# suilin0432/SoS-WSOD

Measured on AMD Instinct MI355X. Metric: images/s (1/2/4/8 MI355X) VGG16+OICR 2000-prop; conv5_3 MFMA-util %, higher is better.
Workload: dtype bf16; 1 GPU; OICR+ training iteration: 4 views/step/GPU (1 image(s) x 2 scales x h-flip, every view 512x512), R=2000 proposals/view, K=20, VGG16 dilated-C5 + ROIPool 7x7 + fc6/fc7 4096 + WSDDN + 4 OICR heads, fwd+bwd+SGD(momentum, wd); image=one view, parallelism=dp1

## Files before the change

### include/soswsod_hip.h

```cpp
#ifndef SOSWSOD_HIP_H
#define SOSWSOD_HIP_H

#include <stdint.h>

#ifdef __cplusplus
extern "C" {
#endif

#ifndef SW_F32
#define SW_F32 0
#define SW_BF16 1
#endif

typedef struct ihipStream_t* sw_stream_t;

typedef struct sw_epilogue {
  const float* bias;
  int relu;
  const uint8_t* drop_mask;
  long ld_drop;
  float drop_scale;
  const void* relu_ref;
  long ld_ref;
  float ref_scale;
// ... 161 lines not shown
typedef struct sw_sgd_tensor_s {
  float* param;
  const float* grad;
  float* momentum_buf;
  long n;
  float lr, weight_decay;
  int first_step;
  int stage_kind, stage_dtype;
  void* stage0;
  void* stage1;
  int d0, d1, d2;
  long ld0, ld1;
  const float* hyper_dev;
} sw_sgd_tensor;
int sw_sgd_multi(int n_tensors, const sw_sgd_tensor* tensors, float momentum, float grad_scale, sw_stream_t stream);
int sw_gemm_sgd_fused_supported(int dtype, int a_kstrided, int b_kstrided, int M, int N, int K);
int sw_loss_finalize(int n_losses, int V, int n_images, const float* loss_view, float* out, float* total,
                     sw_stream_t stream);
int sw_scale_cols_loss(int dtype, int M, int N, int n_valid, const float* in, long ld_in, const float* g_losses,
                       const float* g_total, const int32_t* col_to_loss, float mul, void* out, long ld_out,
                       sw_stream_t stream);
int sw_resize_pass_u8(int C, int H, int W, long in_ld, long in_plane, int out_size, int horizontal, const uint8_t* in,
                      const int32_t* bounds, const int32_t* kk, int ksize, uint8_t* out, uint8_t* out_flip, sw_stream_t stream);
int sw_color_jitter_u8(int H, int W, int mode, const uint8_t* in, float w_bright, double src_w_sat, float w_sat, uint8_t* out,
                       uint8_t* out_flip, sw_stream_t stream);
int sw_pack_views(int R, const float* const* box_ptrs4, const float* const* obj_ptrs4, float* boxes, float* obj,
                  float* rois, sw_stream_t stream);

int sw_preprocess_pad(int dtype, int h, int w, int H, int W, const uint8_t* img_chw, const float* mean3, const float* std3,
                      void* out_nhwc4, sw_stream_t stream);
// ... 157 lines not shown
```

### sos-wsod_amd/_lib.py

```python
import ctypes
import os

import torch

_HERE = os.path.dirname(os.path.abspath(__file__))
LIB_PATH = os.environ.get("SW_LIB_PATH") or os.path.join(_HERE, "libsoswsod_hip.so")

SW_F32, SW_BF16 = 0, 1

c_int, c_long, c_float, c_void_p, c_u64 = ctypes.c_int, ctypes.c_long, ctypes.c_float, ctypes.c_void_p, ctypes.c_uint64
c_int32, c_uint32, c_double, c_longlong = ctypes.c_int32, ctypes.c_uint32, ctypes.c_double, ctypes.c_longlong


class Epilogue(ctypes.Structure):
    _fields_ = [
        ("bias", c_void_p), ("relu", c_int), ("drop_mask", c_void_p), ("ld_drop", c_long), ("drop_scale", c_float),
        ("relu_ref", c_void_p), ("ld_ref", c_long), ("ref_scale", c_float), ("ref_dtype", c_int),
        ("out_dtype", c_int), ("accumulate_atomic", c_int), ("absmax_out", c_void_p),
        ("drop_seed", c_u64), ("drop_offset", c_u64), ("drop_hash_p", c_float), ("drop_offset_dev", c_void_p),
        ("splitk_workspace", c_void_p),
        ("residual", c_void_p), ("ld_res", c_long), ("res_dtype", c_int),
        ("fold_row_scale", c_void_p),
        ("sgd_fused", c_void_p), ("sgd_momentum", c_float), ("sgd_grad_scale", c_float),
    ]
# ... 50 lines not shown
                ("scale", c_void_p), ("shift", c_void_p), ("dst", c_void_p),
                ("kind", c_int32), ("rows", c_int32), ("cols", c_int32), ("block_start", c_int32)]


class ColsumFold(ctypes.Structure):
    _fields_ = [("N", c_int), ("n_partial_rows", c_int), ("workspace", c_void_p), ("out", c_void_p)]


class SgdTensor(ctypes.Structure):
    _fields_ = [
        ("param", c_void_p), ("grad", c_void_p), ("momentum_buf", c_void_p), ("n", c_long), ("lr", c_float),
        ("weight_decay", c_float), ("first_step", c_int), ("stage_kind", c_int), ("stage_dtype", c_int),
        ("stage0", c_void_p), ("stage1", c_void_p), ("d0", c_int), ("d1", c_int), ("d2", c_int), ("ld0", c_long), ("ld1", c_long),
        ("hyper_dev", c_void_p),
    ]


class JpegInfo(ctypes.Structure):
    _fields_ = [("width", c_int32), ("height", c_int32), ("ncomp", c_int32), ("restart_interval", c_int32),
                ("orientation", c_int32), ("mcus_x", c_int32), ("mcus_y", c_int32),
                ("hsamp", c_int32 * 3), ("vsamp", c_int32 * 3), ("qtable", c_int32 * 3),
                ("blocks_w", c_int32 * 3), ("blocks_h", c_int32 * 3), ("coef_bytes", ctypes.c_int64)]


class JpegDesc(ctypes.Structure):
    _fields_ = [("out", c_void_p), ("coef_off", ctypes.c_int64), ("qtab_off", ctypes.c_int64), ("plane_off", ctypes.c_int64),
                ("block_start", c_int32), ("quad_start", c_int32),
                ("width", c_int32), ("height", c_int32), ("ncomp", c_int32), ("hsamp", c_int32), ("vsamp", c_int32),
                ("bgr", c_int32), ("blocks_w", c_int32 * 3), ("blocks_h", c_int32 * 3), ("qtable", c_int32 * 3),
                ("pad_", c_int32)]
# ... 55 lines not shown
    "sw_splitk_fold_multi": (c_int, [c_int, ctypes.POINTER(SplitkFold), c_void_p]),
    "sw_colsum_fold_multi": (c_int, [c_int, ctypes.POINTER(ColsumFold), c_void_p]),
    "sw_colsum_partial_multi": (c_int, [c_int, c_int, ctypes.POINTER(ColsumPart), c_void_p]),
    "sw_conv3x3_wgrad_grouped": (c_int, [c_int, c_int, ctypes.POINTER(WgradProblem), c_void_p]),
    "sw_convert_2d": (c_int, [c_int, c_int, c_int, c_void_p, c_long, c_void_p, c_long, c_void_p]),
    "sw_split_bf16x3": (c_int, [c_int, c_int, c_void_p, c_long, c_void_p, c_long, c_int, c_int, c_void_p]),
    "sw_nchw_to_nhwc": (c_int, [c_int, c_int, c_int, c_int, c_int, c_int, c_void_p, c_void_p, c_void_p]),
    "sw_relu_bwd": (c_int, [c_int, c_long, c_void_p, c_void_p, c_void_p, c_void_p]),
    "sw_scale_cols": (c_int, [c_int, c_int, c_int, c_void_p, c_long, c_void_p, c_void_p, c_long, c_void_p]),
    "sw_fill_zero": (c_int, [c_void_p, c_long, c_void_p]),
    "sw_dropout_mask": (c_int, [c_void_p, c_long, c_u64, c_u64, c_float, c_void_p]),
    "sw_sgd_momentum_step": (c_int, [c_void_p, c_void_p, c_void_p, c_long, c_float, c_float, c_float, c_int, c_float,
                                     c_void_p]),
    "sw_convert_2d_t": (c_int, [c_int, c_int, c_int, c_void_p, c_long, c_void_p, c_long, c_void_p]),
    "sw_sgd_multi": (c_int, [c_int, ctypes.POINTER(SgdTensor), c_float, c_float, c_void_p]),
    "sw_loss_finalize": (c_int, [c_int, c_int, c_int, c_void_p, c_void_p, c_void_p, c_void_p]),
    "sw_scale_cols_loss": (c_int, [c_int, c_int, c_int, c_int, c_void_p, c_long, c_void_p, c_void_p, c_void_p, c_float,
                                   c_void_p, c_long, c_void_p]),
    "sw_resize_pass_u8": (c_int, [c_int, c_int, c_int, c_long, c_long, c_int, c_int, c_void_p, c_void_p, c_void_p, c_int, c_void_p,
                                  c_void_p, c_void_p]),
    "sw_color_jitter_u8": (c_int, [c_int, c_int, c_int, c_void_p, c_float, c_double, c_float, c_void_p, c_void_p, c_void_p]),
    "sw_transpose_2d": (c_int, [c_int, c_int, c_int, c_void_p, c_long, c_void_p, c_long, c_void_p]),
    "sw_stage_blocks": (c_int, [c_int, c_int, c_int]),
    "sw_stage_weights_multi": (c_int, [c_int, c_int, c_void_p, c_int, c_float, c_void_p]),
    "sw_ema_multi": (c_int, [c_int, ctypes.POINTER(c_void_p), ctypes.POINTER(c_void_p), ctypes.POINTER(c_long), c_double, c_void_p]),
    "sw_threshold_select": (c_int, [c_int, c_void_p, c_void_p, c_void_p, c_float, c_void_p, c_int, c_void_p, c_void_p, c_void_p,
                                    c_void_p, c_void_p, c_void_p]),
    "sw_conv3x3_relu_pool2": (c_int, [c_int, c_int, c_int, c_int, c_int, c_int, c_void_p, c_void_p, c_void_p, c_void_p, c_void_p]),
    "sw_weighted_sum": (c_int, [c_int, c_void_p, c_void_p, c_void_p, c_void_p]),
    "sw_scale_scalars": (c_int, [c_int, c_void_p, c_void_p, c_void_p, c_void_p]),
# ... 97 lines not shown
```

### sos-wsod_amd/backbone_vgg.py

```python
import os

import torch
import torch.nn as nn

from . import ops, staging, wgrad
from .registry import BACKBONE_REGISTRY
from .structures import ShapeSpec

_STAGES = [("plain1", 3, 64, 2), ("plain2", 64, 128, 2), ("plain3", 128, 256, 3), ("plain4", 256, 512, 3),
           ("plain5", 512, 512, 3)]


def _epc(dtype):
    return 8 if dtype == torch.bfloat16 else 4


class _Conv(nn.Module):

    def __init__(self, cin, cout):
        super().__init__()
        self.weight = nn.Parameter(torch.empty(cout, cin, 3, 3))
        self.bias = nn.Parameter(torch.zeros(cout))
        nn.init.kaiming_normal_(self.weight, mode="fan_out", nonlinearity="relu")

# ... 134 lines not shown
                w = params[pidx]
                if w.requires_grad:
                    cout = blk.out_channels
                    slab_off, row_off, nslab, nrow, splits = {}, {}, 0, 0, {}
                    for i in live:
                        x_in = infos[i][si][0][ci][0]
                        n, H, W, cin = x_in.shape
                        splits[i] = (direct_ns[(pidx, i)] if direct_ns is not None
                                     else wgrad.wgrad_grouped_splits(nmul * n * H * W, bk, target))
                        slab_off[i], row_off[i] = nslab, nrow
                        nslab += ops.conv3x3_wgrad_nslab_shape(wdt, nmul * n, H, W, cin, cout, splits[i])
                        nrow += ops.colsum_nrows(dtype, n * H * W, cout)
                    cin = infos[live[0]][si][0][ci][0].shape[3]
                    plan[pidx] = dict(ws=torch.empty(nslab, cout * 9 * cin, device=dev, dtype=torch.float32),
                                      rows=torch.empty(nrow, cout, device=dev, dtype=torch.float32), slab_off=slab_off,
                                      row_off=row_off, nslab=nslab, nrow=nrow, splits=splits, cin=cin,
                                      dw=ops.grad_target(w, (cout, cin, 3, 3), dev),
                                      db=ops.grad_target(params[pidx + 1], (cout,), dev))
                if (si, ci) == first_trainable:
                    break
            if si == first_trainable[0]:
                break
        if side is not None:
            side.wait_stream(main)
        for k, i in enumerate(live):
            st = side if (side is not None and k % 2 == 1) else main
            with torch.cuda.stream(st):
                g = gs[i]
                if st is not main:
                    g.record_stream(st)
                _VGGFunction._backward_one(module, infos[i], params, g, dtype, plan, i, first_trainable,
                                           deferred, None if st is main else main, x3w)
            infos[i] = None
        if side is not None:
            main.wait_stream(side)
        if deferred:
            ops.conv3x3_wgrad_grouped(deferred, tag="wgrad_grouped")
            ops.colsum_partial_multi(module._colsum_deferred)
            deferred.clear()
        module._colsum_deferred = []
        ops.conv3x3_wgrad_fold_multi([(pl["ws"], pl["nslab"], pl["dw"]) for pl in plan.values()])
        ops.colsum_fold_multi([(pl["rows"], pl["nrow"], pl["db"]) for pl in plan.values()])
        for pidx, pl in plan.items():
            w = params[pidx]
            grads[pidx] = pl["dw"][:, : w.shape[1]].contiguous() if pl["cin"] != w.shape[1] else pl["dw"]
            grads[pidx + 1] = pl["db"]
        return (None, None) + (None,) * n_in + tuple(grads)

    @staticmethod
    def _backward_one(module, stage_info, params, g, dtype, plan, i, first_trainable, deferred, consumer_stream, x3w=False):
        g = g.contiguous()
        if g.dtype != dtype:
            g = g.to(dtype)
        last_out = stage_info[-1][0][-1][1]
        assert stage_info[-1][1] is None, "backward expects the last stage to have no pool (vgg.py:197)"
        dz = ops.relu_bwd(last_out, g, out=torch.empty_like(g))
        pidx = len(params)
        for si in range(len(stage_info) - 1, -1, -1):
# ... 108 lines not shown
        dtype = self.compute_dtype
        epc = _epc(dtype)
        ft = self.first_trainable_conv()
        for si, blk in enumerate(self.blocks):
            for ci, c in enumerate(blk.convs()):
                cout, cin = c.weight.shape[:2]
                cin_pad = (cin + epc - 1) // epc * epc
                self.staged_weight(c.weight, 0, cin_pad, dtype)
                if self.x3_layer(dtype, cin_pad, cout):
                    self.staged_weight_x3(c.weight, 0, cin_pad)
                if with_dgrad and ft is not None and (si, ci) > ft:
                    self.staged_weight(c.weight, 1, cin, dtype)
                    if self.x3_layer(dtype, cout, cin):
                        self.staged_weight_x3(c.weight, 1, cin)

    def first_trainable_conv(self):
        for si, blk in enumerate(self.blocks):
            for ci, c in enumerate(blk.convs()):
                if c.weight.requires_grad:
                    return (si, ci)
        return None

    def _flat_params(self):
        out = []
        for blk in self.blocks:
            for c in blk.convs():
                out += [c.weight, c.bias]
        return out

    def side_stream(self):
# ... 39 lines not shown
```

### sos-wsod_amd/csrc/common.h

```cpp
#pragma once
#include <hip/hip_runtime.h>
#include <stdint.h>
#include <atomic>

#define SW_F32 0
#define SW_BF16 1

typedef __attribute__((ext_vector_type(4))) float f32x4;
typedef __attribute__((ext_vector_type(16))) float f32x16;
typedef __attribute__((ext_vector_type(8))) __bf16 bf16x8;
typedef __attribute__((ext_vector_type(4))) short s16x4;
typedef __attribute__((ext_vector_type(8))) short s16x8;
typedef __attribute__((ext_vector_type(4))) unsigned int u32x4;
typedef __attribute__((ext_vector_type(2))) unsigned int u32x2;

__device__ __forceinline__ float bf16_bits_to_f32(unsigned short b) {
  return __uint_as_float(((unsigned int)b) << 16);
}
__device__ __forceinline__ unsigned short f32_to_bf16_bits(float f) {
  __bf16 h = (__bf16)f;
  return __builtin_bit_cast(unsigned short, h);
}

template <typename T> struct Elem;
// ... 40 lines not shown
  float r = (lane < nw) ? red[lane] : 0.f;
  r = wave_reduce_sum(r);
  return r;
}
__device__ __forceinline__ float block_reduce_max(float v, float* red) {
  v = wave_reduce_max(v);
  const int lane = threadIdx.x & 63, w = threadIdx.x >> 6, nw = blockDim.x >> 6;
  __syncthreads();
  if (lane == 0) red[w] = v;
  __syncthreads();
  float r = (lane < nw) ? red[lane] : -3.402823466e38f;
  r = wave_reduce_max(r);
  return r;
}

typedef __attribute__((ext_vector_type(4))) int sw_i32x4;
__device__ __forceinline__ sw_i32x4 sw_make_rsrc(const void* base, unsigned bytes) {
  const unsigned long long b = (unsigned long long)base;
  return sw_i32x4{(int)(unsigned)b, (int)(unsigned)((b >> 32) & 0xFFFFu), (int)bytes, 0x00020000};
}
__device__ __forceinline__ void sw_dma16(const sw_i32x4 rsrc, const char* lds_dst, unsigned voff, unsigned soff) {
  const unsigned m = (unsigned)(size_t)(__attribute__((address_space(3))) const char*)lds_dst;
  asm volatile("s_mov_b32 m0, %0\n\ts_nop 0\n\tbuffer_load_dwordx4 %1, %2, %3 offen lds" ::"s"(m), "v"(voff), "s"(rsrc), "s"(soff) : "memory");
}

inline int sw_cu_count() {
  static std::atomic<int> cus[64];
  int dev = 0;
  if (hipGetDevice(&dev) != hipSuccess || dev < 0 || dev >= 64) return 256;
  int n = cus[dev].load(std::memory_order_relaxed);
// ... 14 lines not shown
```

### sos-wsod_amd/csrc/elementwise.hip

```cpp
#include "common.h"
#include "soswsod_hip.h"

namespace {

inline int grid_for(long n, int block = 256) {
  long g = (n + block - 1) / block;
  return (int)(g < 1 ? 1 : (g > 2048 ? 2048 : g));
}

template <typename T>
__global__ void preprocess_kernel(int H, int W, int cpad, const uint8_t* __restrict__ img, float m0, float m1, float m2,
                                  float s0, float s1, float s2, T* __restrict__ out) {
  const long npix = (long)H * W;
  for (long p = blockIdx.x * (long)blockDim.x + threadIdx.x; p < npix; p += (long)gridDim.x * blockDim.x) {
    const float v0 = __fdiv_rn((float)img[p] - m0, s0);
    const float v1 = __fdiv_rn((float)img[npix + p] - m1, s1);
    const float v2 = __fdiv_rn((float)img[2 * npix + p] - m2, s2);
    T* o = out + p * cpad;
    Elem<T>::store(o + 0, v0); Elem<T>::store(o + 1, v1); Elem<T>::store(o + 2, v2);
    for (int c = 3; c < cpad; ++c) Elem<T>::store(o + c, 0.f);
  }
}

constexpr int PRE_MAX = 16;
// ... 321 lines not shown
struct ColsumPartMulti {
  int n;
  int M[CPART_MAX], N[CPART_MAX], rpc[CPART_MAX], slabs[CPART_MAX], first_wg[CPART_MAX + 1];
  long ld[CPART_MAX];
  const void* X[CPART_MAX];
  float* ws[CPART_MAX];
};
template <typename T>
__global__ __launch_bounds__(256) void colsum_ws_multi_kernel(ColsumPartMulti f) {
  int i = 0;
  while (i + 1 < f.n && (int)blockIdx.x >= f.first_wg[i + 1]) ++i;
  const int w = (int)blockIdx.x - f.first_wg[i];
  colsum_ws_body<T>(f.M[i], f.N[i], f.rpc[i], (const T*)f.X[i], f.ld[i], f.ws[i], w % f.slabs[i], w / f.slabs[i]);
}

__device__ __forceinline__ void colsum_fold_body(int N, int nchunk, const float* __restrict__ ws, float* __restrict__ out, int wg,
                                                 const int accumulate = 0) {
  __shared__ float fold[16][17];
  const int tid = threadIdx.x, cl = tid >> 4, c16 = tid & 15, col = wg * 16 + c16;
  float f = 0.f;
  if (col < N)
    for (int c = cl; c < nchunk; c += 16) f += ws[(long)c * N + col];
  fold[cl][c16] = f;
  __syncthreads();
  if (cl == 0 && col < N) {
    float s = 0.f;
#pragma unroll
    for (int r = 0; r < 16; ++r) s += fold[r][c16];
    out[col] = accumulate ? out[col] + s : s;
  }
}

__global__ __launch_bounds__(256) void colsum_fold_kernel(int N, int nchunk, const float* __restrict__ ws, float* __restrict__ out, int accumulate) {
  colsum_fold_body(N, nchunk, ws, out, blockIdx.x, accumulate);
}

constexpr int CFOLD_MAX = 32;
struct ColsumFoldMulti {
  int n;
  int first_wg[CFOLD_MAX + 1];
  int N[CFOLD_MAX], rows[CFOLD_MAX];
  const float* ws[CFOLD_MAX];
  float* out[CFOLD_MAX];
};
__global__ __launch_bounds__(256) void colsum_fold_multi_kernel(ColsumFoldMulti f) {
// ... 39 lines not shown
  if (d.stage_kind == 1) {
    const long r = i / d.d0; const int c = (int)(i - r * d.d0);
    Elem<T>::store((T*)d.stage0 + r * d.ld0 + c, w);
  } else {
    const int tap = (int)(i % 9); const long t = i / 9;
    const int ci = (int)(t % d.d1); const int co = (int)(t / d.d1);
    if (d.stage0) Elem<T>::store((T*)d.stage0 + ((long)co * 9 + tap) * d.d2 + ci, w);
    if (d.stage1) Elem<T>::store((T*)d.stage1 + ((long)ci * 9 + (8 - tap)) * d.d0 + co, w);
  }
}

__device__ __forceinline__ bool sgd_conv_tileable(const sw_sgd_tensor& d) {
  return d.stage_kind == 2 && (d.d0 % 32) == 0 && (d.d1 % 32) == 0;
}

template <typename T>
__device__ __forceinline__ void sgd_conv_tile(const sw_sgd_tensor& d, int blk, float mom, float gscale, float (*tile)[289]) {
  const int cib = d.d1 / 32;
  const int co0 = (blk / cib) * 32, ci0 = (blk % cib) * 32;
  const int Cin = d.d1, Cout = d.d0;
  const float lr = d.hyper_dev ? d.hyper_dev[0] : d.lr, wd = d.hyper_dev ? d.hyper_dev[1] : d.weight_decay;
  for (int idx = threadIdx.x; idx < 32 * 288; idx += 256) {
    const int co_l = idx / 288, rem = idx - co_l * 288;
    const long o = ((long)(co0 + co_l) * Cin + ci0) * 9 + rem;
    const float w0 = d.param[o];
    const float dd = d.grad[o] * gscale + wd * w0;
    const float m = d.first_step ? dd : mom * d.momentum_buf[o] + dd;
    const float w1 = w0 - lr * m;
    d.momentum_buf[o] = m; d.param[o] = w1;
    tile[co_l][rem] = w1;
  }
  __syncthreads();
  if (d.stage0) {
// ... 731 lines not shown
      const long nb = conv_tiles ? (long)(d.d0 / 32) * (d.d1 / 32) : (d.n + SGD_CHUNK - 1) / SGD_CHUNK;
      if (nb > (1L << 30)) return -6;
      b.t[b.n] = d;
      b.block_start[b.n] = blocks;
      blocks += (int)nb;
      ++b.n;
    }
    b.block_start[b.n] = blocks;
    if (b.n == 0) continue;
    hipLaunchKernelGGL(sgd_multi_kernel, dim3(blocks), dim3(256), 0, stream, b, momentum, grad_scale);
    SW_CHECK_LAUNCH();
  }
  return 0;
}

extern "C" int sw_mean_views(int V, long n, const float* in, float* out, hipStream_t stream) {
  SW_ENTER();
  if (n <= 0) return 0;
  hipLaunchKernelGGL(mean_views_kernel, dim3(grid_for(n)), dim3(256), 0, stream, V, n, in, out);
  SW_CHECK_LAUNCH();
  return 0;
}

extern "C" int sw_loss_finalize(int n_losses, int V, int n_images, const float* loss_view, float* out, float* total,
                                hipStream_t stream) {
  SW_ENTER();
  if (n_losses > 64 || n_losses < 1 || V < 1 || n_images < 1) return -6;
  hipLaunchKernelGGL(loss_finalize_kernel, dim3(1), dim3(64), 0, stream, n_losses, V, n_images, loss_view, out, total);
  SW_CHECK_LAUNCH();
  return 0;
// ... 279 lines not shown
```

### sos-wsod_amd/csrc/gemm.hip

```cpp
#include "common.h"
#include "soswsod_hip.h"

namespace {

enum { OP_KCONTIG = 0, OP_KSTRIDED = 1, OP_CONV_A = 2, OP_CONV_B = 3, OP_CONV_A_GEN = 4 };

struct GemmArgs {
  const void* A; const void* B; void* C;
  int M, N, K;
  long lda, ldb, ldc;
  int tiles_m, tiles_n, patches_m, k_per_split;
  int patch_m_log2;
  int cH, cW, cC, cDil;
  const float* bias;
  const uint8_t* drop; long ldd; float drop_scale;
  unsigned long long drop_seed_mixed, drop_offset; float drop_p;
  const unsigned long long* drop_offset_dev;
  const void* ref; long ldr; float ref_scale; int ref_bf16;
  const void* res; long ldres; int res_bf16;
  int relu, out_bf16, atomic, oihw_cin, staged_out;
  unsigned a_bytes, b_bytes;
  long slab_stride;
  int vgrid;
  int krot;
// ... 1125 lines not shown
  return dtype == SW_BF16 ? dispatch_modes<unsigned short>(g, amode, OP_KCONTIG, 1, stream)
                          : dispatch_modes<float>(g, amode, OP_KCONTIG, 1, stream);
}

namespace {
__device__ __forceinline__ void wgrad_reduce_body(int Cout, int Cin, int nslab, const float* __restrict__ slabs,
                                                  float* __restrict__ out, int co, int parts, int part, float* s_t,
                                                  const float* __restrict__ cout_scale = nullptr, const int accumulate = 0) {
  const int CI = Cin / parts, ci0 = part * CI;
  const int cv = CI >> 2, nv = 9 * cv;
  const long slab_f = (long)Cout * 9 * Cin;
  const float* src = slabs + (long)co * 9 * Cin + ci0;
  for (int q = threadIdx.x; q < nv; q += 256) {
    const int tap = q / cv, c4 = q - tap * cv;
    const float* p = src + (long)tap * Cin + c4 * 4;
    f32x4 a0 = {0.f, 0.f, 0.f, 0.f}, a1 = a0, a2 = a0, a3 = a0;
    int z = 0;
    for (; z + 8 <= nslab; z += 8) {
      f32x4 v[8];
#pragma unroll
      for (int u = 0; u < 8; ++u) v[u] = *(const f32x4*)(p + (long)(z + u) * slab_f);
      a0 += v[0]; a1 += v[1]; a2 += v[2]; a3 += v[3];
      a0 += v[4]; a1 += v[5]; a2 += v[6]; a3 += v[7];
    }
    for (; z < nslab; ++z) a0 += *(const f32x4*)(p + (long)z * slab_f);
    f32x4 r = (a0 + a1) + (a2 + a3);
    if (cout_scale) { const float sc = cout_scale[co]; r[0] = __fmul_rn(r[0], sc); r[1] = __fmul_rn(r[1], sc); r[2] = __fmul_rn(r[2], sc); r[3] = __fmul_rn(r[3], sc); }
    *(f32x4*)(s_t + tap * CI + c4 * 4) = r;
  }
  __syncthreads();
  f32x4* dst = (f32x4*)(out + ((long)co * Cin + ci0) * 9);
  for (int q = threadIdx.x; q < nv; q += 256) {
    f32x4 o;
#pragma unroll
    for (int j = 0; j < 4; ++j) {
      const int e = 4 * q + j, ci = e / 9, tap = e - 9 * ci;
      o[j] = s_t[tap * CI + ci];
    }
    if (accumulate) o += dst[q];
    dst[q] = o;
  }
// ... 291 lines not shown
```

### sos-wsod_amd/ops.py

```python
import ctypes

import torch

from ._lib import SW_BF16, SW_F32, Epilogue, check, lib


def _p(t):
    return None if t is None else ctypes.c_void_p(t.data_ptr())


def _floats(vals, n):
    return (ctypes.c_float * n)(*[float(v) for v in vals])


def _workspace256(nbytes, device):
    ws = torch.empty(nbytes + 256, device=device, dtype=torch.uint8)
    return ws, ctypes.c_void_p((ws.data_ptr() + 255) // 256 * 256)


_raw_stream = getattr(torch._C, "_cuda_getCurrentRawStream", None)


def _stream():
    if _raw_stream is not None:
# ... 446 lines not shown
def _fill_sgd_tensor(d, e):
    p = e["param"]
    g = e.get("grad")
    d.param, d.grad, d.momentum_buf, d.n = p.data_ptr(), (None if g is None else g.data_ptr()), e["buf"].data_ptr(), p.numel()
    d.lr, d.weight_decay, d.first_step = float(e["lr"]), float(e["weight_decay"]), int(e["first"])
    hy = e.get("hyper")
    d.hyper_dev = None if hy is None else hy.data_ptr()
    st = e.get("staging")
    if st is None:
        d.stage_kind = 0
    else:
        d.stage_kind, d.stage_dtype = st["kind"], dt(st["dtype"])
        d.stage0 = None if st["stage0"] is None else st["stage0"].data_ptr()
        d.stage1 = None if st["stage1"] is None else st["stage1"].data_ptr()
        d.d0, d.d1, d.d2, d.ld0, d.ld1 = st["d0"], st["d1"], st["d2"], st["ld0"], st.get("ld1", 0)


def gemm_sgd_fused_supported(dtype, M, N, K, a_kstrided=False, b_kstrided=False):
    return bool(lib.sw_gemm_sgd_fused_supported(dt(dtype), int(a_kstrided), int(b_kstrided), int(M), int(N), int(K)))


def attach_sgd_fused(ep, entry, momentum, grad_scale=1.0):
    from ._lib import SgdTensor
    d = SgdTensor()
    _fill_sgd_tensor(d, entry)
    ep.sgd_fused = ctypes.addressof(d)
    ep.sgd_momentum, ep.sgd_grad_scale = float(momentum), float(grad_scale)
    ep._keepalive = ep._keepalive + (d, entry["param"], entry["buf"], entry.get("hyper"))
    return ep

# ... 865 lines not shown
```

### sos-wsod_amd/solver.py

```python
from bisect import bisect_right
from typing import List

import torch

from . import ops, staging


class HipSGD(torch.optim.Optimizer):

    def __init__(self, params, lr, momentum=0.0, weight_decay=0.0, device_hyper=False):
        super().__init__(params, dict(lr=lr, momentum=momentum, weight_decay=weight_decay))
        self.device_hyper = bool(device_hyper)
        self._hyper_dev = None
        self._hyper_host = None
        self._done = set()
        self._group_of = None

    def sync_hyper(self):
        if not self.device_hyper:
            return
        vals = [(float(g["lr"]), float(g["weight_decay"])) for g in self.param_groups]
        if self._hyper_dev is None:
            dev = next(p.device for g in self.param_groups for p in g["params"])
            self._hyper_dev = torch.zeros(len(vals), 2, dtype=torch.float32, device=dev)
# ... 19 lines not shown
        for i, p in enumerate(params):
            g = p.grad if grads is None else grads[i]
            ent = self._group_of.get(id(p))
            if ent is None or g is None or id(p) in self._done:
                continue
            items.append((ent[0], ent[1], p, g.view_as(p)))
            self._done.add(id(p))
        self._update(items, grad_scale)

    @torch.no_grad()
    def fused_update_entry(self, p):
        if self._group_of is None:
            self._group_of = {id(q): (group, gi) for gi, group in enumerate(self.param_groups) for q in group["params"]}
        ent = self._group_of.get(id(p))
        staged = staging.entry_of(p)
        if (ent is None or staged is None or staged["kind"] != 3 or p.dtype != torch.float32 or not p.is_contiguous()):
            return None
        group, gi = ent
        if self.device_hyper and (self._hyper_dev is None or not torch.cuda.is_current_stream_capturing()):
            self.sync_hyper()
        st = self.state[p]
        first = "momentum_buffer" not in st
        if first:
            st["momentum_buffer"] = torch.zeros_like(p, memory_format=torch.contiguous_format)
        entry = dict(param=p, buf=st["momentum_buffer"], lr=group["lr"], weight_decay=group["weight_decay"], first=first,
                     staging=staged, hyper=self._hyper_dev[gi] if self.device_hyper else None)
        return entry, float(group["momentum"]), lambda: staging.updated(p)

    def _update(self, items, grad_scale):
        if not items:
            return
# ... 67 lines not shown
```

### sos-wsod_amd/trainer.py

```python
import os
from collections import OrderedDict

import torch
import torch.distributed as dist

from .events import EventStorage


def init_distributed(backend=None):
    world = int(os.environ.get("WORLD_SIZE", "1"))
    rank = int(os.environ.get("RANK", "0"))
    local_rank = int(os.environ.get("LOCAL_RANK", "0"))
    if world > 1 and not dist.is_initialized():
        if backend is None:
            backend = "nccl" if torch.cuda.is_available() else "gloo"
        if backend == "nccl" and "SW_BENCH_DEVICE" not in os.environ:
            torch.cuda.set_device(local_rank)
        dist.init_process_group(backend=backend, rank=rank, world_size=world)
    return rank, local_rank, world


def auto_scale_workers(cfg, num_workers: int):
    import math
    old = cfg.SOLVER.REFERENCE_WORLD_SIZE
    if old == 0 or old == num_workers or old < num_workers:
        return cfg
    cfg = cfg.clone()
    scale = num_workers / old
    cfg.SOLVER.BASE_LR = cfg.SOLVER.BASE_LR / scale
    cfg.WSL.ITER_SIZE = math.ceil(cfg.WSL.ITER_SIZE / scale)
    return cfg


class Trainer:

    def __init__(self, model, optimizer, data_iter=None, iter_size=1, scheduler=None, ddp=None, find_unused=False,
                 check_finite_every=20, grad_compress=None, metrics_period=20, bucket_cap_mb=128, start_iter=0,
                 use_graph=None, overlap_update=None):
        self.raw_model = model
        self.optimizer, self.scheduler = optimizer, scheduler
        self.iter_size = max(int(iter_size), 1)
        self.data_iter = data_iter
        self.iter = self.start_iter = int(start_iter)
        self.check_finite_every = check_finite_every
        self.metrics_period = metrics_period
        self.storage = EventStorage(self.iter)
        self._finite_flag = None
        self._grad_seed = None
        if use_graph is None:
            use_graph = os.environ.get("SW_STEP_GRAPH", "0") == "1"
        self._graphs = None
        self._want_graph = bool(use_graph)
        self.world = dist.get_world_size() if (dist.is_available() and dist.is_initialized()) else 1
# ... 45 lines not shown
                    def update(fut):
                        v = fut.value()
                        opt.step_params(bucket.parameters(), bucket.gradients())
                        return v[0] if isinstance(v, (list, tuple)) else v
                    return reduce_hook(state, bucket).then(update)
                self.model.register_comm_hook(None, hook)
            else:
                self.model.register_comm_hook(None, reduce_hook)
        else:
            self.model = model
        heads = getattr(model, "roi_heads", None)
        if heads is not None and hasattr(heads, "_fused_fc1_plan"):
            fuse = (not use_ddp and self.iter_size == 1 and hasattr(optimizer, "fused_update_entry")
                    and os.environ.get("SW_FUSE_FC1_UPDATE", "1") == "1")
            heads.__dict__["_fused_opt"] = optimizer if fuse else None
        if self._want_graph and not use_ddp and self.iter_size == 1 and hasattr(model, "roi_heads") and \
                next(model.parameters()).is_cuda:
            self._graphs = _StepGraphs(self)

    def _seed_grad(self, total):
        if self._grad_seed is None or self._grad_seed.device != total.device or self._grad_seed.dtype != total.dtype:
            self._grad_seed = torch.full_like(total, getattr(self, "_seed_scale", 1.0) / self.iter_size)
        return self._grad_seed

    def _raise_if_nonfinite(self):
        if self._finite_flag is not None:
            it, flag = self._finite_flag
            self._finite_flag = None
            if not bool(flag.item()):
                raise FloatingPointError("Loss became infinite or NaN at iteration={}!".format(it))
# ... 465 lines not shown
```

Measured before the change: 499.4 images/s.

## Fuse conv weight-gradient slab fold with SGD update and bf16 weight staging

Adds a grouped kernel that reduces the split-K wgrad slabs and bias partial rows, applies momentum SGD, and writes the staged bf16 (and flipped) weight copies in one pass per 32x32 tile. This replaces the separate fold kernels, gradient materialization and later optimizer/staging passes for backbone convs when running single-GPU with iter_size 1. It also adds a wide vectorized path to the existing conv SGD tile kernel. The fused path drops the separate dw/db tensors, so parameters with existing .grad or unaligned shapes fall back to the old path.

```diff
diff --git a/include/soswsod_hip.h b/include/soswsod_hip.h
--- a/include/soswsod_hip.h
+++ b/include/soswsod_hip.h
@@ -199,6 +199,9 @@
   const float* hyper_dev;
 } sw_sgd_tensor;
 int sw_sgd_multi(int n_tensors, const sw_sgd_tensor* tensors, float momentum, float grad_scale, sw_stream_t stream);
+#define SW_CONV_FOLD_SGD_MAX_ITEMS 24
+typedef struct sw_conv_fold_sgd_item { const float* workspace; int nfold, ws_cin, kind; sw_sgd_tensor t; } sw_conv_fold_sgd_item;
+int sw_conv_fold_sgd_multi(int n, const sw_conv_fold_sgd_item* items, float momentum, float grad_scale, sw_stream_t stream);
 int sw_gemm_sgd_fused_supported(int dtype, int a_kstrided, int b_kstrided, int M, int N, int K);
 int sw_loss_finalize(int n_losses, int V, int n_images, const float* loss_view, float* out, float* total,
                      sw_stream_t stream);
diff --git a/sos-wsod_amd/_lib.py b/sos-wsod_amd/_lib.py
--- a/sos-wsod_amd/_lib.py
+++ b/sos-wsod_amd/_lib.py
@@ -88,6 +88,10 @@
         ("stage0", c_void_p), ("stage1", c_void_p), ("d0", c_int), ("d1", c_int), ("d2", c_int), ("ld0", c_long), ("ld1", c_long),
         ("hyper_dev", c_void_p),
     ]
+
+
+class ConvFoldSgdItem(ctypes.Structure):
+    _fields_ = [("workspace", c_void_p), ("nfold", c_int), ("ws_cin", c_int), ("kind", c_int), ("t", SgdTensor)]
 
 
 class JpegInfo(ctypes.Structure):
@@ -173,6 +177,7 @@
                                      c_void_p]),
     "sw_convert_2d_t": (c_int, [c_int, c_int, c_int, c_void_p, c_long, c_void_p, c_long, c_void_p]),
     "sw_sgd_multi": (c_int, [c_int, ctypes.POINTER(SgdTensor), c_float, c_float, c_void_p]),
+    "sw_conv_fold_sgd_multi": (c_int, [c_int, ctypes.POINTER(ConvFoldSgdItem), c_float, c_float, c_void_p]),
     "sw_loss_finalize": (c_int, [c_int, c_int, c_int, c_void_p, c_void_p, c_void_p, c_void_p]),
     "sw_scale_cols_loss": (c_int, [c_int, c_int, c_int, c_int, c_void_p, c_long, c_void_p, c_void_p, c_void_p, c_float,
                                    c_void_p, c_long, c_void_p]),
diff --git a/sos-wsod_amd/backbone_vgg.py b/sos-wsod_amd/backbone_vgg.py
--- a/sos-wsod_amd/backbone_vgg.py
+++ b/sos-wsod_amd/backbone_vgg.py
@@ -172,9 +172,7 @@
                     cin = infos[live[0]][si][0][ci][0].shape[3]
                     plan[pidx] = dict(ws=torch.empty(nslab, cout * 9 * cin, device=dev, dtype=torch.float32),
                                       rows=torch.empty(nrow, cout, device=dev, dtype=torch.float32), slab_off=slab_off,
-                                      row_off=row_off, nslab=nslab, nrow=nrow, splits=splits, cin=cin,
-                                      dw=ops.grad_target(w, (cout, cin, 3, 3), dev),
-                                      db=ops.grad_target(params[pidx + 1], (cout,), dev))
+                                      row_off=row_off, nslab=nslab, nrow=nrow, splits=splits, cin=cin)
                 if (si, ci) == first_trainable:
                     break
             if si == first_trainable[0]:
@@ -197,9 +195,14 @@
             ops.colsum_partial_multi(module._colsum_deferred)
             deferred.clear()
         module._colsum_deferred = []
-        ops.conv3x3_wgrad_fold_multi([(pl["ws"], pl["nslab"], pl["dw"]) for pl in plan.values()])
-        ops.colsum_fold_multi([(pl["rows"], pl["nrow"], pl["db"]) for pl in plan.values()])
-        for pidx, pl in plan.items():
+        fused = set() if x3w else module._fused_conv_update(params, plan)
+        rest = {pidx: pl for pidx, pl in plan.items() if pidx not in fused}
+        for pidx, pl in rest.items():
+            pl["dw"] = ops.grad_target(params[pidx], (params[pidx].shape[0], pl["cin"], 3, 3), dev)
+            pl["db"] = ops.grad_target(params[pidx + 1], (params[pidx].shape[0],), dev)
+        ops.conv3x3_wgrad_fold_multi([(pl["ws"], pl["nslab"], pl["dw"]) for pl in rest.values()])
+        ops.colsum_fold_multi([(pl["rows"], pl["nrow"], pl["db"]) for pl in rest.values()])
+        for pidx, pl in rest.items():
             w = params[pidx]
             grads[pidx] = pl["dw"][:, : w.shape[1]].contiguous() if pl["cin"] != w.shape[1] else pl["dw"]
             grads[pidx + 1] = pl["db"]
@@ -338,6 +341,31 @@
                     if self.x3_layer(dtype, cout, cin):
                         self.staged_weight_x3(c.weight, 1, cin)
 
+    def _fused_conv_update(self, params, plan):
+        opt = self.__dict__.get("_fused_opt")
+        if opt is None:
+            return set()
+        by_mom = {}
+        for pidx, pl in plan.items():
+            w, b = params[pidx], params[pidx + 1]
+            cout, cin = w.shape[:2]
+            if (pl["cin"] != cin or cout % 32 or cin % 32 or not b.requires_grad or w.grad is not None or b.grad is not None):
+                continue
+            pw = opt.fused_update_entry(w)
+            pb = opt.fused_update_entry(b) if pw is not None else None
+            if pb is None or pw[0]["staging"] is None or pw[0]["staging"]["kind"] != 2 or pw[1] != pb[1]:
+                continue
+            by_mom.setdefault(pw[1], []).append((pidx, pl, pw, pb))
+        fused = set()
+        for mom, group in by_mom.items():
+            rc = ops.conv_fold_sgd_multi([(pl["ws"], pl["nslab"], pl["cin"], pw[0]) for _, pl, pw, _ in group],
+                                         [(pl["rows"], pl["nrow"], pb[0]) for _, pl, _, pb in group], mom)
+            if rc == 0:
+                for pidx, _, pw, pb in group:
+                    pw[2](); pb[2]()
+                    fused.add(pidx)
+        return fused
+
     def first_trainable_conv(self):
         for si, blk in enumerate(self.blocks):
             for ci, c in enumerate(blk.convs()):
diff --git a/sos-wsod_amd/csrc/common.h b/sos-wsod_amd/csrc/common.h
--- a/sos-wsod_amd/csrc/common.h
+++ b/sos-wsod_amd/csrc/common.h
@@ -78,6 +78,36 @@
   return r;
 }
 
+__device__ __forceinline__ f32x4 sw_fold_slabs(const float* __restrict__ p, long slab_f, int nslab) {
+  f32x4 a0 = {0.f, 0.f, 0.f, 0.f}, a1 = a0, a2 = a0, a3 = a0;
+  int z = 0;
+  for (; z + 8 <= nslab; z += 8) {
+    f32x4 v[8];
+#pragma unroll
+    for (int u = 0; u < 8; ++u) v[u] = *(const f32x4*)(p + (long)(z + u) * slab_f);
+    a0 += v[0]; a1 += v[1]; a2 += v[2]; a3 += v[3];
+    a0 += v[4]; a1 += v[5]; a2 += v[6]; a3 += v[7];
+  }
+  if (z + 4 <= nslab) {
+    f32x4 v[4];
+#pragma unroll
+    for (int u = 0; u < 4; ++u) v[u] = *(const f32x4*)(p + (long)(z + u) * slab_f);
+    a0 += v[0]; a0 += v[1]; a0 += v[2]; a0 += v[3];
+    z += 4;
+  }
+  if (z < nslab) {
+    f32x4 v[3];
+#pragma unroll
+    for (int u = 0; u < 3; ++u) v[u] = *(const f32x4*)(p + (long)min(z + u, nslab - 1) * slab_f);
+#pragma unroll
+    for (int u = 0; u < 3; ++u) {
+      const f32x4 t = a0 + v[u];
+      if (z + u < nslab) a0 = t;
+    }
+  }
+  return (a0 + a1) + (a2 + a3);
+}
+
 typedef __attribute__((ext_vector_type(4))) int sw_i32x4;
 __device__ __forceinline__ sw_i32x4 sw_make_rsrc(const void* base, unsigned bytes) {
   const unsigned long long b = (unsigned long long)base;
diff --git a/sos-wsod_amd/csrc/elementwise.hip b/sos-wsod_amd/csrc/elementwise.hip
--- a/sos-wsod_amd/csrc/elementwise.hip
+++ b/sos-wsod_amd/csrc/elementwise.hip
@@ -359,21 +359,27 @@
   colsum_ws_body<T>(f.M[i], f.N[i], f.rpc[i], (const T*)f.X[i], f.ld[i], f.ws[i], w % f.slabs[i], w / f.slabs[i]);
 }
 
-__device__ __forceinline__ void colsum_fold_body(int N, int nchunk, const float* __restrict__ ws, float* __restrict__ out, int wg,
-                                                 const int accumulate = 0) {
-  __shared__ float fold[16][17];
+__device__ __forceinline__ float colsum_fold_sum(int N, int nchunk, const float* __restrict__ ws, int wg, float (*fold)[17]) {
   const int tid = threadIdx.x, cl = tid >> 4, c16 = tid & 15, col = wg * 16 + c16;
   float f = 0.f;
   if (col < N)
     for (int c = cl; c < nchunk; c += 16) f += ws[(long)c * N + col];
   fold[cl][c16] = f;
   __syncthreads();
+  float s = 0.f;
   if (cl == 0 && col < N) {
-    float s = 0.f;
 #pragma unroll
     for (int r = 0; r < 16; ++r) s += fold[r][c16];
-    out[col] = accumulate ? out[col] + s : s;
-  }
+  }
+  return s;
+}
+
+__device__ __forceinline__ void colsum_fold_body(int N, int nchunk, const float* __restrict__ ws, float* __restrict__ out, int wg,
+                                                 const int accumulate = 0) {
+  __shared__ float fold[16][17];
+  const int col = wg * 16 + (threadIdx.x & 15);
+  const float s = colsum_fold_sum(N, nchunk, ws, wg, fold);
+  if ((threadIdx.x >> 4) == 0 && col < N) out[col] = accumulate ? out[col] + s : s;
 }
 
 __global__ __launch_bounds__(256) void colsum_fold_kernel(int N, int nchunk, const float* __restrict__ ws, float* __restrict__ out, int accumulate) {
@@ -443,9 +449,87 @@
   return d.stage_kind == 2 && (d.d0 % 32) == 0 && (d.d1 % 32) == 0;
 }
 
+__device__ __forceinline__ void sgd_elem(float w0, float g, float mbuf, int first, float lr, float wd, float mom, float gscale,
+                                         float& m, float& w1) {
+  const float dd = g * gscale + wd * w0;
+  m = first ? dd : mom * mbuf + dd;
+  w1 = w0 - lr * m;
+}
+
+__device__ __forceinline__ void store4(float* p, const float (&v)[4]) { *(f32x4*)p = f32x4{v[0], v[1], v[2], v[3]}; }
+__device__ __forceinline__ void store4(unsigned short* p, const float (&v)[4]) {
+  *(u32x2*)p = u32x2{(unsigned)f32_to_bf16_bits(v[0]) | ((unsigned)f32_to_bf16_bits(v[1]) << 16),
+                     (unsigned)f32_to_bf16_bits(v[2]) | ((unsigned)f32_to_bf16_bits(v[3]) << 16)};
+}
+
+template <bool FOLDED>
+__device__ __forceinline__ void conv_tile_update(float* __restrict__ param, float* __restrict__ mbuf, const float* __restrict__ grad,
+                                                 int Cin, int co0, int ci0, int first, float lr, float wd, float mom, float gscale,
+                                                 float (*tile)[289]) {
+#pragma unroll 3
+  for (int it = 0; it < 9; ++it) {
+    const int q = (int)threadIdx.x + it * 256;
+    const int co_l = q / 72, rem = (q - co_l * 72) * 4;
+    const long o = ((long)(co0 + co_l) * Cin + ci0) * 9 + rem;
+    const f32x4 w4 = *(const f32x4*)(param + o);
+    f32x4 g4;
+    if (FOLDED) g4 = f32x4{tile[co_l][rem], tile[co_l][rem + 1], tile[co_l][rem + 2], tile[co_l][rem + 3]};
+    else g4 = *(const f32x4*)(grad + o);
+    f32x4 b4 = {0.f, 0.f, 0.f, 0.f};
+    if (!first) b4 = *(const f32x4*)(mbuf + o);
+    f32x4 m4, n4;
+#pragma unroll
+    for (int e = 0; e < 4; ++e) {
+      float m, w1;
+      sgd_elem(w4[e], g4[e], b4[e], first, lr, wd, mom, gscale, m, w1);
+      m4[e] = m; n4[e] = w1;
+      tile[co_l][rem + e] = w1;
+    }
+    *(f32x4*)(mbuf + o) = m4;
+    *(f32x4*)(param + o) = n4;
+  }
+}
+
+template <typename T>
+__device__ __forceinline__ void conv_tile_stage(T* __restrict__ s0, T* __restrict__ s1, int Cout, int d2, int co0, int ci0,
+                                                const float (*tile)[289]) {
+  if (s0) {
+#pragma unroll 3
+    for (int it = 0; it < 9; ++it) {
+      const int q = (int)threadIdx.x + it * 256;
+      const int run = q >> 3, c4 = (q & 7) * 4, co_l = run / 9, tap = run - co_l * 9;
+      const float v[4] = {tile[co_l][c4 * 9 + tap], tile[co_l][(c4 + 1) * 9 + tap], tile[co_l][(c4 + 2) * 9 + tap],
+                          tile[co_l][(c4 + 3) * 9 + tap]};
+      store4(s0 + ((long)(co0 + co_l) * 9 + tap) * d2 + ci0 + c4, v);
+    }
+  }
+  if (s1) {
+#pragma unroll 3
+    for (int it = 0; it < 9; ++it) {
+      const int q = (int)threadIdx.x + it * 256;
+      const int run = q >> 3, c4 = (q & 7) * 4, ci_l = run / 9, tapf = run - ci_l * 9, e = ci_l * 9 + (8 - tapf);
+      const float v[4] = {tile[c4][e], tile[c4 + 1][e], tile[c4 + 2][e], tile[c4 + 3][e]};
+      store4(s1 + ((long)(ci0 + ci_l) * 9 + tapf) * Cout + co0 + c4, v);
+    }
+  }
+}
+
+__device__ __forceinline__ bool sgd_conv_wide(const sw_sgd_tensor& d) {
+  return (((uintptr_t)d.param | (uintptr_t)d.grad | (uintptr_t)d.momentum_buf | (uintptr_t)d.stage0 | (uintptr_t)d.stage1) & 15) == 0 &&
+         (d.d2 % 4) == 0;
+}
+
 template <typename T>
 __device__ __forceinline__ void sgd_conv_tile(const sw_sgd_tensor& d, int blk, float mom, float gscale, float (*tile)[289]) {
   const int cib = d.d1 / 32;
+  if (sgd_conv_wide(d)) {
+    const int co0 = (blk / cib) * 32, ci0 = (blk % cib) * 32;
+    const float lr = d.hyper_dev ? d.hyper_dev[0] : d.lr, wd = d.hyper_dev ? d.hyper_dev[1] : d.weight_decay;
+    conv_tile_update<false>(d.param, d.momentum_buf, d.grad, d.d1, co0, ci0, d.first_step, lr, wd, mom, gscale, tile);
+    __syncthreads();
+    conv_tile_stage<T>((T*)d.stage0, (T*)d.stage1, d.d0, d.d2, co0, ci0, tile);
+    return;
+  }
   const int co0 = (blk / cib) * 32, ci0 = (blk % cib) * 32;
   const int Cin = d.d1, Cout = d.d0;
   const float lr = d.hyper_dev ? d.hyper_dev[0] : d.lr, wd = d.hyper_dev ? d.hyper_dev[1] : d.weight_decay;
@@ -1207,6 +1291,106 @@
   return 0;
 }
 
+namespace {
+constexpr int CFS_MAX = SW_CONV_FOLD_SGD_MAX_ITEMS;
+struct ConvFoldSgdItem {
+  const float* ws;
+  float* param;
+  float* mbuf;
+  void* stage0;
+  void* stage1;
+  const float* hyper;
+  int nfold, d0, d1, d2, first, stage_dtype, kind;
+  float lr, wd;
+};
+struct ConvFoldSgdBatch {
+  ConvFoldSgdItem it[CFS_MAX];
+  int block_start[CFS_MAX + 1];
+  int n;
+};
+
+__global__ __launch_bounds__(256) void conv_fold_sgd_multi_kernel(ConvFoldSgdBatch b, float mom, float gscale) {
+  __shared__ float tile[32][289];
+  __shared__ float fold[16][17];
+  int i = 0;
+  while (i + 1 < b.n && (int)blockIdx.x >= b.block_start[i + 1]) ++i;
+  const ConvFoldSgdItem& d = b.it[i];
+  const int blk = (int)blockIdx.x - b.block_start[i];
+  const float lr = d.hyper ? d.hyper[0] : d.lr, wd = d.hyper ? d.hyper[1] : d.wd;
+  if (d.kind == 1) {
+    const int col = blk * 16 + ((int)threadIdx.x & 15);
+    const float s = colsum_fold_sum(d.d0, d.nfold, d.ws, blk, fold);
+    if ((threadIdx.x >> 4) == 0 && col < d.d0) {
+      float m, w1;
+      sgd_elem(d.param[col], s, d.first ? 0.f : d.mbuf[col], d.first, lr, wd, mom, gscale, m, w1);
+      d.mbuf[col] = m; d.param[col] = w1;
+    }
+    return;
+  }
+  const int Cout = d.d0, Cin = d.d1, cib = Cin / 32;
+  const int co0 = (blk / cib) * 32, ci0 = (blk % cib) * 32;
+  const long slab_f = (long)Cout * 9 * Cin;
+#pragma unroll 3
+  for (int it = 0; it < 9; ++it) {
+    const int q = (int)threadIdx.x + it * 256;
+    const int run = q >> 3, c4 = (q & 7) * 4, co_l = run / 9, tap = run - co_l * 9;
+    const f32x4 r = sw_fold_slabs(d.ws + ((long)(co0 + co_l) * 9 + tap) * Cin + ci0 + c4, slab_f, d.nfold);
+#pragma unroll
+    for (int j = 0; j < 4; ++j) tile[co_l][(c4 + j) * 9 + tap] = r[j];
+  }
+  __syncthreads();
+  conv_tile_update<true>(d.param, d.mbuf, nullptr, Cin, co0, ci0, d.first, lr, wd, mom, gscale, tile);
+  __syncthreads();
+  if (d.stage_dtype == SW_BF16) conv_tile_stage<unsigned short>((unsigned short*)d.stage0, (unsigned short*)d.stage1, Cout, d.d2, co0, ci0, tile);
+  else conv_tile_stage<float>((float*)d.stage0, (float*)d.stage1, Cout, d.d2, co0, ci0, tile);
+}
+}
+
+extern "C" int sw_conv_fold_sgd_multi(int n, const sw_conv_fold_sgd_item* items, float momentum, float grad_scale,
+                                      hipStream_t stream) {
+  SW_ENTER();
+  static_assert(sizeof(float) * (32 * 289 + 16 * 17) <= 65536, "the tile and the bias fold share one workgroup's 64 KiB of LDS");
+  static_assert(sizeof(ConvFoldSgdBatch) + 8 <= 4096, "the descriptors travel in the kernel arguments");
+  for (int i = 0; i < n; ++i) {
+    const sw_conv_fold_sgd_item& q = items[i];
+    const sw_sgd_tensor& t = q.t;
+    if (q.nfold < 1 || !q.workspace || !t.param || !t.momentum_buf) return -5;
+    if (q.kind == 1) {
+      if (t.n <= 0 || t.n > (1L << 24) || t.stage_kind != 0) return -5;
+      if ((((uintptr_t)q.workspace) | ((uintptr_t)t.param) | ((uintptr_t)t.momentum_buf) | ((uintptr_t)t.hyper_dev)) & 3) return -4;
+      continue;
+    }
+    if (q.kind != 0 || t.stage_kind != 2) return -1;
+    if (t.stage_dtype != SW_BF16 && t.stage_dtype != SW_F32) return -1;
+    if (t.d0 <= 0 || t.d1 <= 0 || (t.d0 % 32) || (t.d1 % 32) || (long)t.d0 * t.d1 * 9 != t.n) return -5;
+    if (q.ws_cin != t.d1) return -5;
+    if (t.stage0 && (t.d2 < t.d1 || (t.d2 % 4))) return -5;
+    if ((long)(t.d0 / 32) * (t.d1 / 32) > (1L << 24)) return -6;
+    if ((((uintptr_t)q.workspace) | ((uintptr_t)t.param) | ((uintptr_t)t.momentum_buf) | ((uintptr_t)t.stage0) | ((uintptr_t)t.stage1)) & 15)
+      return -4;
+    if (((uintptr_t)t.hyper_dev) & 3) return -4;
+  }
+  for (int base = 0; base < n; base += CFS_MAX) {
+    ConvFoldSgdBatch b = {};
+    b.n = n - base < CFS_MAX ? n - base : CFS_MAX;
+    long blocks = 0;
+    for (int i = 0; i < b.n; ++i) {
+      const sw_conv_fold_sgd_item& q = items[base + i];
+      const sw_sgd_tensor& t = q.t;
+      ConvFoldSgdItem& o = b.it[i];
+      o.ws = q.workspace; o.param = t.param; o.mbuf = t.momentum_buf; o.stage0 = t.stage0; o.stage1 = t.stage1; o.hyper = t.hyper_dev;
+      o.nfold = q.nfold; o.kind = q.kind; o.first = t.first_step; o.stage_dtype = t.stage_dtype; o.lr = t.lr; o.wd = t.weight_decay;
+      if (q.kind == 1) { o.d0 = (int)t.n; o.d1 = o.d2 = 0; } else { o.d0 = t.d0; o.d1 = t.d1; o.d2 = t.d2; }
+      b.block_start[i] = (int)blocks;
+      blocks += q.kind == 1 ? (t.n + 15) / 16 : (long)(t.d0 / 32) * (t.d1 / 32);
+    }
+    b.block_start[b.n] = (int)blocks;
+    hipLaunchKernelGGL(conv_fold_sgd_multi_kernel, dim3((unsigned)blocks), dim3(256), 0, stream, b, momentum, grad_scale);
+    SW_CHECK_LAUNCH();
+  }
+  return 0;
+}
+
 extern "C" int sw_mean_views(int V, long n, const float* in, float* out, hipStream_t stream) {
   SW_ENTER();
   if (n <= 0) return 0;
diff --git a/sos-wsod_amd/csrc/gemm.hip b/sos-wsod_amd/csrc/gemm.hip
--- a/sos-wsod_amd/csrc/gemm.hip
+++ b/sos-wsod_amd/csrc/gemm.hip
@@ -1163,17 +1163,7 @@
   for (int q = threadIdx.x; q < nv; q += 256) {
     const int tap = q / cv, c4 = q - tap * cv;
     const float* p = src + (long)tap * Cin + c4 * 4;
-    f32x4 a0 = {0.f, 0.f, 0.f, 0.f}, a1 = a0, a2 = a0, a3 = a0;
-    int z = 0;
-    for (; z + 8 <= nslab; z += 8) {
-      f32x4 v[8];
-#pragma unroll
-      for (int u = 0; u < 8; ++u) v[u] = *(const f32x4*)(p + (long)(z + u) * slab_f);
-      a0 += v[0]; a1 += v[1]; a2 += v[2]; a3 += v[3];
-      a0 += v[4]; a1 += v[5]; a2 += v[6]; a3 += v[7];
-    }
-    for (; z < nslab; ++z) a0 += *(const f32x4*)(p + (long)z * slab_f);
-    f32x4 r = (a0 + a1) + (a2 + a3);
+    f32x4 r = sw_fold_slabs(p, slab_f, nslab);
     if (cout_scale) { const float sc = cout_scale[co]; r[0] = __fmul_rn(r[0], sc); r[1] = __fmul_rn(r[1], sc); r[2] = __fmul_rn(r[2], sc); r[3] = __fmul_rn(r[3], sc); }
     *(f32x4*)(s_t + tap * CI + c4 * 4) = r;
   }
diff --git a/sos-wsod_amd/ops.py b/sos-wsod_amd/ops.py
--- a/sos-wsod_amd/ops.py
+++ b/sos-wsod_amd/ops.py
@@ -484,6 +484,23 @@
         d.stage0 = None if st["stage0"] is None else st["stage0"].data_ptr()
         d.stage1 = None if st["stage1"] is None else st["stage1"].data_ptr()
         d.d0, d.d1, d.d2, d.ld0, d.ld1 = st["d0"], st["d1"], st["d2"], st["ld0"], st.get("ld1", 0)
+
+
+def conv_fold_sgd_multi(weights, biases, momentum, grad_scale=1.0):
+    from ._lib import ConvFoldSgdItem
+    n = len(weights) + len(biases)
+    if n == 0:
+        return 0
+    arr = (ConvFoldSgdItem * n)()
+    for i, (ws, nfold, ws_cin, e) in enumerate([(w[0], w[1], w[2], w[3]) for w in weights] + [(b[0], b[1], 0, b[2]) for b in biases]):
+        _need_gpu(ws, e["param"], e["buf"])
+        q = arr[i]
+        q.workspace, q.nfold, q.ws_cin, q.kind = ws.data_ptr(), int(nfold), int(ws_cin), int(i >= len(weights))
+        _fill_sgd_tensor(q.t, e)
+    rc = lib.sw_conv_fold_sgd_multi(n, arr, float(momentum), float(grad_scale), _stream())
+    if rc > 0:
+        check(rc, "sw_conv_fold_sgd_multi")
+    return rc
 
 
 def gemm_sgd_fused_supported(dtype, M, N, K, a_kstrided=False, b_kstrided=False):
diff --git a/sos-wsod_amd/solver.py b/sos-wsod_amd/solver.py
--- a/sos-wsod_amd/solver.py
+++ b/sos-wsod_amd/solver.py
@@ -57,7 +57,8 @@
             self._group_of = {id(q): (group, gi) for gi, group in enumerate(self.param_groups) for q in group["params"]}
         ent = self._group_of.get(id(p))
         staged = staging.entry_of(p)
-        if (ent is None or staged is None or staged["kind"] != 3 or p.dtype != torch.float32 or not p.is_contiguous()):
+        takes = (staged["kind"] in (2, 3)) if staged is not None else p.dim() == 1
+        if ent is None or not takes or p.dtype != torch.float32 or not p.is_contiguous():
             return None
         group, gi = ent
         if self.device_hyper and (self._hyper_dev is None or not torch.cuda.is_current_stream_capturing()):
diff --git a/sos-wsod_amd/trainer.py b/sos-wsod_amd/trainer.py
--- a/sos-wsod_amd/trainer.py
+++ b/sos-wsod_amd/trainer.py
@@ -34,9 +34,11 @@
 
 class Trainer:
 
+    FUSE_CONV_UPDATE = True
+
     def __init__(self, model, optimizer, data_iter=None, iter_size=1, scheduler=None, ddp=None, find_unused=False,
                  check_finite_every=20, grad_compress=None, metrics_period=20, bucket_cap_mb=128, start_iter=0,
-                 use_graph=None, overlap_update=None):
+                 use_graph=None, overlap_update=None, fuse_conv_update=None):
         self.raw_model = model
         self.optimizer, self.scheduler = optimizer, scheduler
         self.iter_size = max(int(iter_size), 1)
@@ -112,6 +114,12 @@
             fuse = (not use_ddp and self.iter_size == 1 and hasattr(optimizer, "fused_update_entry")
                     and os.environ.get("SW_FUSE_FC1_UPDATE", "1") == "1")
             heads.__dict__["_fused_opt"] = optimizer if fuse else None
+        backbone = getattr(model, "backbone", None)
+        if backbone is not None and hasattr(backbone, "_fused_conv_update"):
+            if fuse_conv_update is None:
+                fuse_conv_update = self.FUSE_CONV_UPDATE
+            fuse = bool(fuse_conv_update) and not use_ddp and self.iter_size == 1 and hasattr(optimizer, "fused_update_entry")
+            backbone.__dict__["_fused_opt"] = optimizer if fuse else None
         if self._want_graph and not use_ddp and self.iter_size == 1 and hasattr(model, "roi_heads") and \
                 next(model.parameters()).is_cuda:
             self._graphs = _StepGraphs(self)
```

After: 501.8 images/s (median of 6 runs). Within noise of the previous version (+0.5%).
